# david-cortes/cmfrec

Hardware: AMD Instinct MI355X
Metric: ALS rows/sec ((users+items)/iteration time), implicit ALS-CG k=50 fp64 (higher is better)
Workload: dtype f64

## Files before the change

cmfrec_amd/csrc/cg_kernels.hpp:

```cpp
#pragma once
#include <hip/hip_runtime.h>
#include <stdint.h>
#include <type_traits>

#include "lanes.hpp"

namespace cmfhip {

constexpr int WAVE = 64;
constexpr int TILE = 64;
constexpr int MAX_W = 8;
#ifndef CMF_CG_WAVES_PER_SIMD
#define CMF_CG_WAVES_PER_SIMD 2
#endif
#ifndef CMF_CG_WAVES_PER_SIMD_F32
#define CMF_CG_WAVES_PER_SIMD_F32 3
#endif
#ifndef CMF_CG_WAVES_PER_SIMD_LOW
#define CMF_CG_WAVES_PER_SIMD_LOW 3
#endif
constexpr int CG_NTSEL_MAX_S = 7;
template <typename T, int W, int NRES_, int NTSEL = 0> constexpr int cg_waves_per_simd()
{
    if (sizeof(T) == 8 && NTSEL == 1 && W <= 8) return CMF_CG_WAVES_PER_SIMD_LOW;
// ... 110 lines not shown
#pragma unroll
        for (int s = 0; s < S; s++) tile.set(t, s, val);
}

template <typename T>
__device__ __forceinline__ T wave_sum(T v) { return lanes::wave_sum(v); }

template <typename T, int NT, int I>
__device__ __forceinline__ T treduce8_low_first(const T (&v)[8], bool h)
{
    if constexpr (I + 4 < NT) {
        T keep = h ? v[I + 4] : v[I];
        return keep + lanes::recv_xor4(v[I], v[I + 4]);
    } else return v[I] + lanes::xor4_lower(v[I]);
}
template <typename T, int NT = 8>
__device__ __forceinline__ T treduce8_low(const T (&v)[8], int lane)
{
    static_assert(NT >= 4 && NT <= 8, "entries per lane group");
    T u[4], q[2];
    bool h = (lane & 4) != 0;
    u[0] = treduce8_low_first<T, NT, 0>(v, h); u[1] = treduce8_low_first<T, NT, 1>(v, h);
    u[2] = treduce8_low_first<T, NT, 2>(v, h); u[3] = treduce8_low_first<T, NT, 3>(v, h);
    h = (lane & 2) != 0;
#pragma unroll
    for (int i = 0; i < 2; i++) {
        T keep = h ? u[i + 2] : u[i];
        T send = h ? u[i] : u[i + 2];
        q[i] = keep + lanes::xor2(send);
    }
    h = (lane & 1) != 0;
    T keep = h ? q[1] : q[0];
    T send = h ? q[0] : q[1];
    return keep + lanes::xor1(send);
}

template <typename T>
__device__ __forceinline__ T treduce8_high(const T (&v)[8], int lane)
{
    T u[4], q[2];
#pragma unroll
    for (int i = 0; i < 4; i++) u[i] = lanes::tswap32_add(v[i], v[i + 4]);
#pragma unroll
    for (int i = 0; i < 2; i++) q[i] = lanes::tswap16_add(u[i], u[i + 2]);
    const bool h = (lane & 8) != 0;
    T keep = h ? q[1] : q[0];
    return keep + lanes::recv_xor8(q[0], q[1]);
}

#ifndef CMF_PASS_VECTOR_LDS
#define CMF_PASS_VECTOR_LDS 2
#endif
template <typename T> constexpr bool pass_vector_in_lds() { return CMF_PASS_VECTOR_LDS == 1 || (CMF_PASS_VECTOR_LDS == 2 && sizeof(T) == 8); }
template <typename T, int S>
__device__ __forceinline__ void replicate(T vdist, T (&vrep)[S], int lane);
template <typename T, int S, int GR = 8>
__device__ __forceinline__ void pass_vector_lds(T vdist, T (&vrep)[S], T (&wts)[8], int lane, T *__restrict__ pv)
{
    const int jj = lane >> 3, ll = lane & 7;
    pv[lane] = vdist;
    __builtin_amdgcn_wave_barrier();
#pragma unroll
    for (int s = 0; s < S; s++) vrep[s] = pv[ll + 8 * s];
    const T *wp = pv + GR * jj;
#pragma unroll
    for (int t = 0; t < GR; t++) wts[t] = wp[t];
    __builtin_amdgcn_wave_barrier();
}

__host__ __device__ constexpr int gram_ld(int S) { return 8 * S + 1; }
#ifndef CMF_GRAM_ROWS_BY_K
#define CMF_GRAM_ROWS_BY_K 1
#endif
template <typename T> __host__ __device__ constexpr int gram_rows(int S) { return (CMF_GRAM_ROWS_BY_K && pass_vector_in_lds<T>()) ? S : 8; }
__host__ __device__ constexpr int gram_ld_rows(int S, int GR)
{
    if (GR == 8) return gram_ld(S);
    int ld = 8 * S;
    while ((S * ld) % 32 != 8 && (S * ld) % 32 != 24) ld++;
    return ld;
}
__host__ __device__ constexpr int gram_ld2(int S) { return 8 * S + 2; }
template <typename T> __host__ __device__ constexpr int gram_elems(int S) { return sizeof(T) == 4 ? 64 * gram_ld2(S) : 64 * gram_ld(S); }
template <typename T, int S, int GR = 8> __device__ __forceinline__ int gram_index(int r, int c)
{
    if constexpr (sizeof(T) == 4) return 2 * ((r >> 1) * gram_ld2(S) + c) + (r & 1);
    else return r * gram_ld_rows(S, GR) + c;
}
template <typename T, int S, int GR = 8>
__device__ __forceinline__ void stage_gramian(T *__restrict__ G, const T *__restrict__ BtB, int k, int tid, int nthreads)
{
    static_assert(GR == 8 || sizeof(T) == 8, "rows by k: double precision");
    for (int e = tid; e < 8 * GR * 8 * S; e += nthreads) {
        const int r = e / (8 * S), c = e % (8 * S);
        G[gram_index<T, S, GR>(r, c)] = (r < k && c < k) ? BtB[(size_t)r * k + c] : T(0);
    }
}

template <typename T, int S>
struct RegTile {
    T v[8][S];
    __device__ __forceinline__ void set(int t, int s, T x) { v[t][s] = x; }
};
typedef float f32x2 __attribute__((ext_vector_type(2)));
template <int S>
struct RegTile<float, S> {
    f32x2 v[4][S];
    __device__ __forceinline__ void set(int t, int s, float x) { v[t >> 1][s][t & 1] = x; }
};

template <typename T>
struct PassAcc {
    T v[8];
    __device__ __forceinline__ void zero()
    {
#pragma unroll
        for (int s = 0; s < 8; s++) v[s] = T(0);
    }
    __device__ __forceinline__ void close(T (&out)[8]) const
    {
#pragma unroll
        for (int s = 0; s < 8; s++) out[s] = v[s];
    }
};
template <>
struct PassAcc<float> {
    f32x2 v[8];
    __device__ __forceinline__ void zero()
    {
#pragma unroll
        for (int s = 0; s < 8; s++) v[s] = f32x2{0.f, 0.f};
    }
    __device__ __forceinline__ void close(float (&out)[8]) const
    {
#pragma unroll
        for (int s = 0; s < 8; s++) out[s] = v[s][0] + v[s][1];
    }
};

template <typename T, int S, int NT = 8>
__device__ __forceinline__ void load_tile(RegTile<T, S> &tile, const T *__restrict__ Bm, size_t ldb,
                                          int k, int my_idx, int cnt, int lane)
{
    const int jj = lane >> 3, ll = lane & 7;
    int its[8];
    its[0] = lanes::bcast8<0>(my_idx); its[1] = lanes::bcast8<1>(my_idx); its[2] = lanes::bcast8<2>(my_idx);
    its[3] = lanes::bcast8<3>(my_idx);
    if (NT > 4) its[4] = lanes::bcast8<4>(my_idx);
    if (NT > 5) its[5] = lanes::bcast8<5>(my_idx);
    if (NT > 6) its[6] = lanes::bcast8<6>(my_idx);
    if (NT > 7) its[7] = lanes::bcast8<7>(my_idx);
    const int first_idx = __builtin_amdgcn_readfirstlane(my_idx);
    const int col_last = min(ll + 8 * (S - 1), k - 1) - ll;
    const char *base = reinterpret_cast<const char *>(Bm + ll);
    const unsigned ldb_bytes = (unsigned)(ldb * sizeof(T));
#pragma unroll
    for (int t = 0; t < NT; t++) {
        const unsigned it = (unsigned)(((jj * NT + t) < cnt) ? its[t] : first_idx);
        const T *rp = reinterpret_cast<const T *>(base + (unsigned long long)it * ldb_bytes);
#pragma unroll
        for (int s = 0; s < S; s++) tile.set(t, s, rp[(s < S - 1) ? 8 * s : col_last]);
    }
}

template <typename T, bool IMPLICIT, int MODE>
__device__ __forceinline__ T pass_weight(T coef, T x, bool valid, T g = T(1))
// ... 85 lines not shown
        for (int s = S; s < 8; s++) out.v[s] = T(0);
    }
    }
}

template <typename T, int S, int W>
__device__ __forceinline__ void gram_pass(const T *__restrict__ G, T wdist, PassAcc<T> &out, int lane, int wr)
{
    constexpr int LD = gram_ld(S);
    const int jj = lane >> 3, ll = lane & 7;
    T wts[8];
    wts[0] = lanes::bcast8<0>(wdist); wts[1] = lanes::bcast8<1>(wdist); wts[2] = lanes::bcast8<2>(wdist);
    wts[3] = lanes::bcast8<3>(wdist); wts[4] = lanes::bcast8<4>(wdist); wts[5] = lanes::bcast8<5>(wdist);
    wts[6] = lanes::bcast8<6>(wdist); wts[7] = lanes::bcast8<7>(wdist);
    if constexpr (std::is_same<T, float>::value && W <= 4) {
#pragma unroll
        for (int q = 0; q < 4; q++) {
            if (W > 1 && (q % W) != wr) continue;
            const f32x2 *g = reinterpret_cast<const f32x2 *>(G) + (jj * 4 + q) * gram_ld2(S) + ll;
            const f32x2 w2 = f32x2{wts[2 * q], wts[2 * q + 1]};
#pragma unroll
            for (int s = 0; s < S; s++) out.v[s] += w2 * lds_g(g + 8 * s);
        }
    } else {
#pragma unroll
        for (int t = 0; t < 8; t++) {
            if (W > 1 && (t % W) != wr) continue;
#pragma unroll
            for (int s = 0; s < S; s++) {
                if constexpr (std::is_same<T, float>::value) out.v[s][0] += wts[t] * G[gram_index<T, S>(jj * 8 + t, ll + 8 * s)];
                else out.v[s] += wts[t] * lds_g(G + (jj * 8 + t) * LD + ll + 8 * s);
            }
        }
    }
}

template <bool NEG, typename T, int S, int W, int GR = 8>
__device__ __forceinline__ void gram_pass_w(const T *__restrict__ G, const T (&wts)[8], PassAcc<T> &out, int lane, int wr)
{
    constexpr int LD = gram_ld_rows(S, GR);
    const int jj = lane >> 3, ll = lane & 7;
    if constexpr (std::is_same<T, float>::value && W <= 4) {
#pragma unroll
        for (int q = 0; q < 4; q++) {
            if (W > 1 && (q % W) != wr) continue;
            const f32x2 *g = reinterpret_cast<const f32x2 *>(G) + (jj * 4 + q) * gram_ld2(S) + ll;
            const f32x2 w2 = f32x2{wts[2 * q], wts[2 * q + 1]};
#pragma unroll
            for (int s = 0; s < S; s++) out.v[s] = NEG ? out.v[s] - w2 * lds_g(g + 8 * s) : out.v[s] + w2 * lds_g(g + 8 * s);
        }
    } else {
#pragma unroll
        for (int t = 0; t < GR; t++) {
            if (W > 1 && (t % W) != wr) continue;
#pragma unroll
            for (int s = 0; s < S; s++) {
                if constexpr (std::is_same<T, float>::value) {
                    const float g = G[gram_index<T, S>(jj * 8 + t, ll + 8 * s)];
                    out.v[s][0] = NEG ? out.v[s][0] - wts[t] * g : out.v[s][0] + wts[t] * g;
                } else {
                    const T g = lds_g(G + (jj * GR + t) * LD + ll + 8 * s);
                    out.v[s] = NEG ? out.v[s] - wts[t] * g : out.v[s] + wts[t] * g;
                }
            }
        }
    }
}

template <typename T, int S>
__device__ __forceinline__ void replicate(T vdist, T (&vrep)[S], int lane)
{
    const int ll = lane & 7;
#pragma unroll
    for (int s = 0; s < S; s++) vrep[s] = __shfl(vdist, s * 8 + ll);
}

template <typename T, int S, bool IMPLICIT, int W, int RPB, bool GRAMX = false, int NRES_ = 0, int NTSEL = 0>
__global__ void __launch_bounds__(64 * W * RPB, (cg_waves_per_simd<T, W, NRES_, NTSEL>()))
cg_rows_kernel(const CgParams<T> P)
{
    constexpr bool GRAM = IMPLICIT || GRAMX;
    extern __shared__ __attribute__((aligned(16))) unsigned char smem_raw[];
    T *G = reinterpret_cast<T *>(smem_raw);
    T *red = G + (GRAM ? gram_elems<T>(S) : 0);
    const int tid = threadIdx.x;
    const int lane = tid & 63;
    const int wave = tid >> 6;
    const int grp = wave / W;
    const int wr = wave % W;
    const int k = P.k;

    const int nteams = gridDim.x * RPB;
    __shared__ int s_claim[4];
    constexpr bool PV = pass_vector_in_lds<T>();
    __shared__ __attribute__((aligned(16))) T s_pv[PV ? W * RPB : 1][PV ? 64 : 1];
    const int cslot = (blockIdx.x * RPB + grp) % CG_NCOUNTERS;
    int *const my_counter = P.counter + cslot * CG_COUNTER_STRIDE;
    const int cbase = nteams + cslot;
    auto issue_claim = [&]() -> int {
        int v = 0;
        if (wr == 0 && lane == 0) v = atomicAdd(my_counter, 1);
        return v;
    };
    int rnxt, rnn;
    if (W == 1) {
        const int c1 = issue_claim(), c2 = issue_claim();
        rnxt = cbase + CG_NCOUNTERS * __builtin_amdgcn_readfirstlane(c1);
        rnn = cbase + CG_NCOUNTERS * __builtin_amdgcn_readfirstlane(c2);
    } else if (wr == 0 && lane == 0) {
        s_claim[2] = cbase + CG_NCOUNTERS * atomicAdd(my_counter, 1);
        s_claim[3] = cbase + CG_NCOUNTERS * atomicAdd(my_counter, 1);
    }
    constexpr int GR = gram_rows<T>(S);
    if (GRAM) stage_gramian<T, S, GR>(G, P.BtB, k, tid, blockDim.x);
    if (GRAM || W > 1) __syncthreads();
    if (W > 1) { rnxt = s_claim[2]; rnn = s_claim[3]; }
    T *myred = red + (size_t)grp * 2 * W * 64;

    int buf = 0;
    static_assert(W == 1 || RPB == 1, "multi-wave teams own their workgroup (barriers are per row)");

    constexpr int NRES = NRES_ > 0 ? NRES_ : ((std::is_same<T, float>::value && W == 8) ? 2 : 1);
    static_assert(NRES == 1 || std::is_same<T, float>::value, "two resident tiles: single precision");
    static_assert(NTSEL == 0 || (S >= CMF_CG_NT_MIN_S && (sizeof(T) == 4 || S <= CG_NTSEL_MAX_S) && NRES_ == 0),
                  "launches by tile size: tiles by row length (double precision: k <= 56)");
    constexpr int NT_MIN = (S >= CMF_CG_NT_MIN_S && (CMF_CG_NT_F32 || !std::is_same<T, float>::value)) ? (std::is_same<T, float>::value ? 6 : 5) : 8;
    auto nt_of = [&](int nnz_) -> int {
        int nt = (nnz_ + 8 * W * NRES - 1) / (8 * W * NRES);
        if (std::is_same<T, float>::value) nt = (nt + 1) & ~1;
        return (nt > 8) ? 8 : (nt < NT_MIN ? NT_MIN : nt);
    };
    struct Pre { int idx; T x; T a; int idx2; T x2; T g; T g2; };
    auto load_desc = [&](int rix_) -> RowDesc {
        RowDesc d; d.row = 0; d.nnz = 0; d.st = 0;
        if (rix_ < P.nrows) d = P.desc[rix_];
        d.row = __builtin_amdgcn_readfirstlane(d.row);
        d.nnz = __builtin_amdgcn_readfirstlane(d.nnz);
        d.st = ((unsigned long long)(unsigned)__builtin_amdgcn_readfirstlane((int)(d.st >> 32)) << 32) |
               (unsigned)__builtin_amdgcn_readfirstlane((int)(d.st & 0xffffffffu));
        return d;
    };
    auto load_pre = [&](const RowDesc &d) -> Pre {
        Pre q; q.idx = 0; q.x = T(0); q.a = T(0); q.idx2 = 0; q.x2 = T(0); q.g = T(1); q.g2 = T(1);
        const int nt = nt_of(d.nnz), tl = 8 * nt;
        const int b = lane & 7;
        const int ent = (lane >> 3) * nt + b;
        const int cnt = min(tl, d.nnz - wr * tl);
        if (b < nt && ent < cnt) {
            const size_t pos = d.st + (size_t)wr * tl + ent;
            q.idx = P.indices[pos];
            q.x = P.values[pos];
            q.g = entry_weight<T, IMPLICIT>(P, pos);
            if (!IMPLICIT && P.bias_sub != nullptr) q.x -= P.bias_sub[q.idx];
        }
        if (NRES == 2) {
            const int cnt2 = min(tl, d.nnz - (wr + W) * tl);
            if (b < nt && ent < cnt2) {
                const size_t pos = d.st + (size_t)(wr + W) * tl + ent;
                q.idx2 = P.indices[pos];
                q.x2 = P.values[pos];
                q.g2 = entry_weight<T, IMPLICIT>(P, pos);
                if (!IMPLICIT && P.bias_sub != nullptr) q.x2 -= P.bias_sub[q.idx2];
            }
        }
        if (d.nnz > 0 && lane < k) q.a = P.A[(size_t)d.row * P.lda + lane];
        return q;
    };
    int rix = blockIdx.x * RPB + grp;
    RowDesc dcur = load_desc(rix);
    RowDesc dnxt = load_desc(rnxt);
    Pre pcur = load_pre(dcur);
    int pend = issue_claim();
#ifdef CMF_CG_TICKS
    unsigned long long tk_wait = 0, tk_pass = 0, tk_rows = 0;
    const unsigned long long tk_begin = CMF_TICK();
#endif
    int it = 0;
    RowDesc dnn;
    Pre pnxt;
    auto solve_row = [&](auto nt_tag) {
        constexpr int NT = decltype(nt_tag)::value;
        constexpr int TL = 8 * NT;
        const int row = dcur.row;
        const size_t st = dcur.st;
        const int nnz = dcur.nnz;
        const int ntiles = (nnz + TL - 1) / TL;
        const int my_ntiles = (ntiles > wr) ? (ntiles - wr + W - 1) / W : 0;
        const bool resident = NT < 8 || my_ntiles <= NRES;

        T lam = P.lam, lam_last = P.lam_last;
        if (GRAMX && P.kc > 0) {
            if (P.scale_lam || P.scale_lam_sideinfo) {
                T mult = row_lam_mult(P, row, nnz);
                if (P.scale_lam_sideinfo) mult += (T)P.p_side;
                lam *= mult; lam_last *= mult;
            }
        } else if (!IMPLICIT && P.scale_lam) {
            const T mult = row_lam_mult(P, row, nnz);
            lam *= mult;
            if (!P.scale_bias_const) lam_last *= mult;
        }
        T *arow = P.A + (size_t)row * P.lda;
        T a_d = pcur.a;

        RegTile<T, S> tile;
        const int ent = (lane >> 3) * NT + (lane & 7);
        const bool lane_has = (NT == 8) || (lane & 7) < NT;
        const int cnt0 = min(TL, nnz - wr * TL);
        T x_res = pcur.x;
        const T g_res = pcur.g;
        bool valid_res = lane_has && ent < cnt0;
        if (CMF_DBG(P, 1)) dbg_fill_tile<8, S>(tile, (T)(pcur.idx & 3) * (T)0.001);
        else if (cnt0 > 0) load_tile<T, S, NT>(tile, P.B, P.ldb, k, pcur.idx, cnt0, lane);
        RegTile<T, (NRES == 2) ? S : 1> tile2;
        const int cnt1 = (NRES == 2) ? min(TL, nnz - (wr + W) * TL) : 0;
        const T x2_res = pcur.x2, g2_res = pcur.g2;
        const bool valid2_res = lane_has && ent < cnt1;
        if constexpr (NRES == 2) {
            if (cnt1 > 0 && !CMF_DBG(P, 1)) load_tile<T, S, NT>(tile2, P.B, P.ldb, k, pcur.idx2, cnt1, lane);
        }
        dnn = load_desc(rnn);
        pnxt = load_pre(dnxt);
#ifdef CMF_CG_TICKS
        const unsigned long long tk0 = CMF_TICK();
        asm volatile("s_waitcnt vmcnt(0)" ::: "memory");
        const unsigned long long tk1 = CMF_TICK();
        tk_wait += tk1 - tk0;
#endif

        auto run_pass = [&](T vdist, auto mode_tag, bool first) -> T {
            constexpr int MODE = decltype(mode_tag)::value;
            asm volatile("" ::: "memory");
            T vrep[S];
            T gw[8];
            if constexpr (PV) pass_vector_lds<T, S, GR>(vdist, vrep, gw, lane, &s_pv[wave][0]);
            else replicate<T, S>(vdist, vrep, lane);
            PassAcc<T> acc;
            acc.zero();
            if constexpr (NRES == 2) {
                if (cnt0 > 0 && !CMF_DBG(P, 4)) tile_pass<T, S, IMPLICIT, MODE, NT>(tile, vrep, x_res, valid_res, acc, lane, g_res);
                if (cnt1 > 0 && !CMF_DBG(P, 4)) tile_pass<T, S, IMPLICIT, MODE, NT>(tile2, vrep, x2_res, valid2_res, acc, lane, g2_res);
            } else if constexpr (NT < 8) {
                if (cnt0 > 0 && !CMF_DBG(P, 4)) tile_pass<T, S, IMPLICIT, MODE, NT>(tile, vrep, x_res, valid_res, acc, lane, g_res);
            } else
            for (int tl = wr; tl < ntiles; tl += W) {
                T x, g; bool valid;
                const bool have = (tl == wr) && (resident || first);
                if (!have) {
                    const int cnt = min(TL, nnz - tl * TL);
                    valid = lane_has && ent < cnt;
                    const size_t pos = st + (size_t)tl * TL + ent;
                    int my_idx = valid ? P.indices[pos] : 0;
                    x = valid ? P.values[pos] : T(0);
                    g = valid ? entry_weight<T, IMPLICIT>(P, pos) : T(1);
                    if (!IMPLICIT && P.bias_sub != nullptr && valid) x -= P.bias_sub[my_idx];
                    if (!CMF_DBG(P, 1)) load_tile<T, S, NT>(tile, P.B, P.ldb, k, my_idx, cnt, lane);
                } else {
                    x = x_res; g = g_res; valid = valid_res;
                }
                if (!CMF_DBG(P, 4)) tile_pass<T, S, IMPLICIT, MODE, NT>(tile, vrep, x, valid, acc, lane, g);
            }
            if (GRAM && !CMF_DBG(P, 2)) {
                if constexpr (PV) gram_pass_w<MODE == 0, T, S, W, GR>(G, gw, acc, lane, wr);
                else gram_pass<T, S, W>(G, (MODE == 0) ? -vdist : vdist, acc, lane, wr);
            }
            T out[8];
            acc.close(out);
            T tot = treduce8_high<T>(out, lane);
            if (W > 1) {
                T *rb = myred + (size_t)buf * W * 64;
                rb[wr * 64 + lane] = tot;
                if (first && wr == 0 && lane == 0) s_claim[it & 1] = cbase + CG_NCOUNTERS * pend;
                __syncthreads();
                tot = T(0);
#pragma unroll
                for (int w = 0; w < W; w++) tot += rb[w * 64 + lane];
                buf ^= 1;
            }
            return tot;
        };

        T r_d = run_pass(a_d, std::integral_constant<int, 0>{}, true);
        r_d -= lam * a_d;
        if (!IMPLICIT && lam != lam_last && lane == k - 1) r_d -= (lam_last - lam) * a_d;
        if (GRAMX && P.rconst != nullptr && lane < k) r_d += P.rconst[(size_t)row * P.ldr + lane];
        if (lane >= k) r_d = T(0);
        T p_d = r_d;
        T r_old = CMF_DBG(P, 8) ? T(1) : wave_sum(r_d * r_d);
        bool done = (r_old <= (T)1e-12);
        for (int step = 0; step < P.max_cg_steps && !done; step++) {
            T Ap_d = run_pass(p_d, std::integral_constant<int, 1>{}, false);
            Ap_d += lam * p_d;
            if (!IMPLICIT && lam != lam_last && lane == k - 1) Ap_d += (lam_last - lam) * p_d;
            if (lane >= k) Ap_d = T(0);
            T alpha = CMF_DBG(P, 8) ? T(0.001) : cg_div(r_old, wave_sum(Ap_d * p_d));
            a_d += alpha * p_d;
            r_d -= alpha * Ap_d;
            T r_new = CMF_DBG(P, 8) ? T(0.5) : wave_sum(r_d * r_d);
            if (r_new <= (T)1e-8) done = true;
            else {
                p_d = p_d * cg_div(r_new, r_old) + r_d;
                r_old = r_new;
            }
        }
        if (wr == 0 && lane < k) arow[lane] = a_d;
#ifdef CMF_CG_TICKS
        tk_pass += CMF_TICK() - tk1; tk_rows += (wr == 0);
#endif
    };
    for (; rix < P.nrows; it++) {
        const int nt = nt_of(dcur.nnz);
        if constexpr (NT_MIN == 8) solve_row(std::integral_constant<int, 8>{});
        else if constexpr (std::is_same<T, float>::value) {
            if constexpr (NTSEL == 1) solve_row(std::integral_constant<int, 6>{});
            else if constexpr (NTSEL == 2) solve_row(std::integral_constant<int, 8>{});
            else if (nt == 6) solve_row(std::integral_constant<int, 6>{});
            else solve_row(std::integral_constant<int, 8>{});
        } else if constexpr (NTSEL == 1) {
            if (nt <= 5) solve_row(std::integral_constant<int, 5>{});
            else solve_row(std::integral_constant<int, 6>{});
        } else if constexpr (NTSEL == 2) {
            if (nt <= 7) solve_row(std::integral_constant<int, 7>{});
            else solve_row(std::integral_constant<int, 8>{});
        } else {
            switch (nt) {
                case 5: solve_row(std::integral_constant<int, 5>{}); break;
                case 6: solve_row(std::integral_constant<int, 6>{}); break;
                case 7: solve_row(std::integral_constant<int, 7>{}); break;
                default: solve_row(std::integral_constant<int, 8>{}); break;
            }
        }
        const int r3 = (W == 1) ? cbase + CG_NCOUNTERS * __builtin_amdgcn_readfirstlane(pend) : s_claim[it & 1];
        dcur = dnxt; dnxt = dnn; pcur = pnxt;
        rix = rnxt; rnxt = rnn; rnn = r3;
        pend = issue_claim();
    }
#ifdef CMF_CG_TICKS
    cg_ticks_flush(P.ticks, W == 1 ? 0 : W == 2 ? 1 : W == 4 ? 2 : 3, tk_wait, tk_pass, tk_rows, CMF_TICK() - tk_begin, lane);
#endif
}

constexpr int TILE4 = 32;

template <typename T, int S>
struct RegTile4 {
    T v[4][S];
    __device__ __forceinline__ void set(int t, int s, T x) { v[t][s] = x; }
    __device__ __forceinline__ T get(int t, int s) const { return v[t][s]; }
};
template <int S>
struct RegTile4<float, S> {
    f32x2 v[2][S];
    __device__ __forceinline__ void set(int t, int s, float x) { v[t >> 1][s][t & 1] = x; }
    __device__ __forceinline__ f32x2 pair0(int s) const { return v[0][s]; }
};

template <typename T, int S>
__device__ __forceinline__ void load_tile4(RegTile4<T, S> &tile, const T *__restrict__ Bm, size_t ldb,
                                           int k, int my_idx, int cnt, int lane)
{
    const int jj = lane >> 3, ll = lane & 7;
    int its[4];
    its[0] = lanes::bcast8<0>(my_idx); its[1] = lanes::bcast8<2>(my_idx);
    its[2] = lanes::bcast8<4>(my_idx); its[3] = lanes::bcast8<6>(my_idx);
    const int first_idx = __builtin_amdgcn_readfirstlane(my_idx);
    const int col_last = min(ll + 8 * (S - 1), k - 1) - ll;
    const char *base = reinterpret_cast<const char *>(Bm + ll);
    const unsigned ldb_bytes = (unsigned)(ldb * sizeof(T));
#pragma unroll
    for (int t = 0; t < 4; t++) {
        const unsigned it = (unsigned)(((jj * 4 + t) < cnt) ? its[t] : first_idx);
        const T *rp = reinterpret_cast<const T *>(base + (unsigned long long)it * ldb_bytes);
#pragma unroll
        for (int s = 0; s < S; s++) tile.set(t, s, rp[(s < S - 1) ? 8 * s : col_last]);
    }
}

template <typename T>
__device__ __forceinline__ T treduce4_low(const T (&v)[4], int lane)
{
    T u[2];
    bool h = (lane & 4) != 0;
#pragma unroll
    for (int i = 0; i < 2; i++) {
        T keep = h ? v[i + 2] : v[i];
        u[i] = keep + lanes::recv_xor4(v[i], v[i + 2]);
    }
    h = (lane & 2) != 0;
    T keep = h ? u[1] : u[0];
    T send = h ? u[0] : u[1];
    T q = keep + lanes::xor2(send);
    return q + lanes::xor1(q);
}

template <int S, bool IMPLICIT, int MODE, typename TILE, bool INIT = false>
__device__ __forceinline__ void tile_pass4_f32(const TILE &tile, const float (&vrep)[S], float x, bool valid,
                                           PassAcc<float> &out, int lane, float g = 1.f)
{
    float c[4];
#pragma unroll
    for (int q = 0; q < 2; q++) {
        f32x2 acc = f32x2{0.f, 0.f};
#pragma unroll
        for (int s = 0; s < S; s++) acc += tile.v[q][s] * f32x2{vrep[s], vrep[s]};
        c[2 * q] = acc[0]; c[2 * q + 1] = acc[1];
    }
    float coef = treduce4_low<float>(c, lane);
    const float w = pass_weight<float, IMPLICIT, MODE>(coef, x, valid, g);
    float wts[4];
    wts[0] = lanes::bcast8<0>(w); wts[1] = lanes::bcast8<2>(w); wts[2] = lanes::bcast8<4>(w); wts[3] = lanes::bcast8<6>(w);
#pragma unroll
    for (int q = 0; q < 2; q++) {
        const f32x2 w2 = f32x2{wts[2 * q], wts[2 * q + 1]};
#pragma unroll
        for (int s = 0; s < S; s++) out.v[s] = (INIT && q == 0) ? w2 * tile.v[q][s] : out.v[s] + w2 * tile.v[q][s];
    }
    if constexpr (INIT) {
#pragma unroll
// ... 854 lines not shown
```

cmfrec_amd/csrc/device.hpp:

```cpp
#pragma once
#include <hip/hip_runtime.h>
#include <algorithm>
#include <cstdio>
#include <cstdlib>
#include <cstring>
#include <numeric>
#include <string>
#include <vector>

#include "../../include/cmfrec_hip.h"
#include "cg_kernels.hpp"
#include "chol_kernels.hpp"
#include "dense_kernels.hpp"
#include "gram_cg_kernels.hpp"
#include "topn_kernels.hpp"

namespace cmfhip {

extern thread_local std::string g_last_error;

struct HipError {
    int code;
};

inline void hip_check(hipError_t e, const char *what, const char *file, int line)
{
    if (e == hipSuccess) return;
    char buf[512];
    snprintf(buf, sizeof buf, "cmfrec_hip: %s failed: %s (%s:%d)", what, hipGetErrorString(e), file, line);
    g_last_error = buf;
    fprintf(stderr, "%s\n", buf);
    throw HipError{e == hipErrorOutOfMemory ? 1 : 4};
}
#define HIP_CHECK(x) ::cmfhip::hip_check((x), #x, __FILE__, __LINE__)

struct Switches {
    bool poison_lds = false;
    int vh_min = 0;
    int vh = 0;
    bool gram_slice = false;
    int bins_par = 2;
    bool nt_split = true;
    bool cg_generic = false;
    int chol = 0;
    int parts_coop = 1;
    int chol_wg = 2;
    int gramk = -1;
    int gramk_batch = 0;
    int lowrank = -1;
    bool eig_jacobi = false;
    int debug_skip = 0;
    bool debug_ticks = false;
    void reload()
    {
        auto str = [](const char *n) -> const char * { const char *v = getenv(n); return (v != nullptr && v[0] != 0) ? v : nullptr; };
        auto num = [&](const char *n, int dflt) -> int { const char *v = str(n); return v ? atoi(v) : dflt; };
        poison_lds = str("CMFREC_HIP_POISON_LDS") != nullptr;
        vh_min = num("CMFREC_HIP_VH_MIN", 0);
        const char *v = str("CMFREC_HIP_VH");
        vh = !v ? 0 : strcmp(v, "stream") == 0 ? 1 : strcmp(v, "gram") == 0 ? 2 : 1;
        v = str("CMFREC_HIP_GRAM_KERNEL"); gram_slice = v && strcmp(v, "slice") == 0;
        bins_par = num("CMFREC_HIP_BINS_PAR", 2);
        nt_split = num("CMFREC_HIP_NT_SPLIT", 1) != 0;
        v = str("CMFREC_HIP_CG_KERNEL"); cg_generic = v && strcmp(v, "generic") == 0;
        v = str("CMFREC_HIP_CHOL"); chol = !v ? 0 : strcmp(v, "rows") == 0 ? 1 : strcmp(v, "noslices") == 0 ? 2 : 0;
        parts_coop = num("CMFREC_HIP_PARTS_COOP", 1);
        chol_wg = num("CMFREC_HIP_CHOL_WG", 2);
        if (chol_wg == 1) chol_wg = 2;
        gramk = num("CMFREC_HIP_GRAMK", -1);
        gramk_batch = num("CMFREC_HIP_GRAMK_BATCH", 0);
        lowrank = num("CMFREC_HIP_LOWRANK", -1);
        v = str("CMFREC_HIP_EIG"); eig_jacobi = v && strcmp(v, "jacobi") == 0;
        debug_skip = num("CMFREC_HIP_CG_SKIP", num("CMFREC_HIP_CHOL_SKIP", num("CMFREC_HIP_WAVE_SKIP", 0)));
        debug_ticks = str("CMFREC_HIP_GRAM_TICKS") != nullptr || str("CMFREC_HIP_CHOL_TICKS") != nullptr;
    }
};
inline Switches &switches_mut() { static Switches sw; static bool first = (sw.reload(), true); (void)first; return sw; }
inline const Switches &switches() { return switches_mut(); }

template <typename T>
struct DevBuf {
    T *ptr = nullptr;
    size_t n = 0;
    bool owned = true;
    DevBuf() = default;
    DevBuf(const DevBuf &) = delete;
    DevBuf &operator=(const DevBuf &) = delete;
    ~DevBuf() { release(); }
    void release()
    {
        if (ptr && owned) (void)hipFree(ptr);
        ptr = nullptr;
        n = 0;
    }
    void alloc(size_t count)
    {
        release();
        n = count;
        owned = true;
        if (count) HIP_CHECK(hipMalloc((void **)&ptr, count * sizeof(T)));
        if (count && switches().poison_lds) {
            HIP_CHECK(hipMemset(ptr, 0xFF, count * sizeof(T)));
            HIP_CHECK(hipDeviceSynchronize());
        }
    }
    void alloc_at_least(size_t count)
    {
        if (n < count) alloc(count);
    }
    void upload(const T *host, size_t count, hipStream_t st)
    {
        if (count > n) alloc(count);
        if (count) HIP_CHECK(hipMemcpyAsync(ptr, host, count * sizeof(T), hipMemcpyDefault, st));
    }
    void download(T *host, size_t count, hipStream_t st) const
    {
        if (count) HIP_CHECK(hipMemcpyAsync(host, ptr, count * sizeof(T), hipMemcpyDeviceToHost, st));
    }
};

constexpr int MAX_DEVICES = 16;
constexpr int NBINS = 6;
constexpr int BIN_VHEAVY = 0;
constexpr int BIN_HEAVY = 1;
constexpr int BIN_MED4 = 2;
constexpr int BIN_MED2 = 3;
constexpr int BIN_LIGHT = 4;
constexpr int BIN_TINY = 5;
constexpr int BIN_MIN_NNZ[NBINS] = {1025, 257, 129, 65, 33, 1};
inline int vh_min_env()
{
    const int v = switches().vh_min;
    return v > 0 ? std::min(sizeof(real_t) == 4 ? BIN_MIN_NNZ[BIN_VHEAVY] : (1 << 30), std::max(258, v)) : 0;
}

struct SparseShard {
    int nrows = 0;
    size_t nnz = 0;
    int vh_min = BIN_MIN_NNZ[BIN_VHEAVY];
    size_t opp_row_bytes_hint = 50 * sizeof(real_t);
    int bin_of(long long l) const
    {
        if (l >= vh_min) return BIN_VHEAVY;
        for (int b = 1; b < NBINS; b++)
            if (l >= BIN_MIN_NNZ[b]) return b;
        return -1;
// ... 313 lines not shown
        }
        hipLaunchKernelGGL(gram_reduce_kernel<real_t>, dim3((k * k + GRAM_RED_ENT - 1) / GRAM_RED_ENT), dim3(256), 0, dev.stream,
                           ws.partial.ptr, nblocks, k * k, out, scale, add_diag, k);
    } else {
        launch_gemm<true>(dev, k, k, n, scale, B, ldb, B, ldb, out, (size_t)k);
        if (add_diag != 0)
            hipLaunchKernelGGL(add_diag_kernel<real_t>, dim3((k + 255) / 256), dim3(256), 0, dev.stream, out, k, 0, k, add_diag);
    }
    HIP_CHECK(hipGetLastError());
}

struct CgCall {
    real_t *A; size_t lda;
    const real_t *B; size_t ldb;
    int k;
    const real_t *bias_sub;
    const real_t *BtB;
    real_t lam, lam_last;
    bool scale_lam, scale_bias_const;
    int max_cg_steps;
    bool implicit;
    bool precond = false;
    int koff = 0, kc = 0;
    const real_t *CtC = nullptr, *UC = nullptr;
    real_t w_side = 0;
    int rows_with_u = 0, p_side = 0;
    bool scale_lam_sideinfo = false;
    const SparseShard *X2 = nullptr;
    const real_t *C2 = nullptr;
    const real_t *Bi = nullptr, *BiTBi = nullptr;
    int ki = 0;
    real_t w_imp = 0;
    const real_t *gsum = nullptr;
    int skip_first = 0;
    const real_t *Gx = nullptr, *rconst_x = nullptr;
    size_t ldr_x = 0;
    const real_t *values_override = nullptr, *weights_override = nullptr;
    bool gx_all_rows = false;
    const real_t *wsum_override = nullptr;
};

enum class CgVariant { Auto, Generic };
CgVariant cg_variant_from_env();

constexpr int NCOUNTER_SETS = 2 * NBINS + 2;
constexpr size_t ROW_COUNTER_INTS = 64 + (size_t)NCOUNTER_SETS * CG_NCOUNTERS * CG_COUNTER_STRIDE;
inline size_t cg_counter_offset(int bin) { return 64 + (size_t)bin * CG_NCOUNTERS * CG_COUNTER_STRIDE; }

__global__ void __launch_bounds__(256) poison_lds_kernel(int words)
{
    extern __shared__ unsigned int poison_words[];
    volatile unsigned int *w = poison_words;
    for (int e = threadIdx.x; e < words; e += 256) w[e] = 0xFFFFFFFFu;
}
inline void poison_lds(hipStream_t st, int num_cus)
{
    if (!switches().poison_lds) return;
    constexpr int BYTES = 80 * 1024;
    static thread_local bool attr_set = false;
    if (!attr_set) {
        HIP_CHECK(hipFuncSetAttribute((const void *)poison_lds_kernel, hipFuncAttributeMaxDynamicSharedMemorySize, BYTES));
        attr_set = true;
    }
    hipLaunchKernelGGL(poison_lds_kernel, dim3(num_cus * 4), dim3(256), BYTES, st, BYTES / 4);
    HIP_CHECK(hipGetLastError());
}

template <int S, bool IMPLICIT, int W, int RPB, bool GRAMX = false, int NRES_ = 0, int NTSEL = 0>
inline void launch_cg_bin(const DeviceInfo &dev, CgParams<real_t> P, int first, int count, BinTimers *tm, int bin, hipStream_t st, int counter_set = -1)
{
    if (count <= 0) return;
    EventPair ev{nullptr, nullptr};
    if (tm) {
        HIP_CHECK(hipEventCreate(&ev.a));
        HIP_CHECK(hipEventCreate(&ev.b));
        HIP_CHECK(hipEventRecord(ev.a, st));
    }
    poison_lds(st, dev.num_cus);
    P.order += first;
    P.desc += first;
    P.nrows = count;
    P.counter = dev.row_counter.ptr + cg_counter_offset(counter_set >= 0 ? counter_set : bin);
    constexpr int threads = 64 * W * RPB;
    size_t smem = (((IMPLICIT || GRAMX) ? (size_t)gram_elems<real_t>(S) : 0) + (size_t)RPB * 2 * W * 64) * sizeof(real_t);
    auto kern = cg_rows_kernel<real_t, S, IMPLICIT, W, RPB, GRAMX, NRES_, NTSEL>;
    static thread_local int bpc_dev[MAX_DEVICES] = {0};
    int &blocks_per_cu = bpc_dev[std::min(std::max(dev.device, 0), MAX_DEVICES - 1)];
    if (blocks_per_cu == 0) {
        if (smem > 48 * 1024)
            HIP_CHECK(hipFuncSetAttribute((const void *)kern, hipFuncAttributeMaxDynamicSharedMemorySize, (int)smem));
        int nb = 0;
        HIP_CHECK(hipOccupancyMaxActiveBlocksPerMultiprocessor(&nb, kern, threads, smem));
        blocks_per_cu = std::max(1, nb);
    }
    int teams_needed = (count + RPB - 1) / RPB;
    int grid = std::min(teams_needed, dev.num_cus * blocks_per_cu);
    hipLaunchKernelGGL(kern, dim3(grid), dim3(threads), smem, st, P);
    HIP_CHECK(hipGetLastError());
    if (tm) {
        HIP_CHECK(hipEventRecord(ev.b, st));
        tm->ev[bin].push_back(ev);
    }
}

template <int S, bool IMPLICIT, bool GRAMX = false>
inline void launch_cg_tiny(const DeviceInfo &dev, CgParams<real_t> P, int first, int count, BinTimers *tm, hipStream_t st, int n_gt16)
{
    if (count <= 0) return;
    EventPair ev{nullptr, nullptr};
    if (tm) {
        HIP_CHECK(hipEventCreate(&ev.a));
        HIP_CHECK(hipEventCreate(&ev.b));
        HIP_CHECK(hipEventRecord(ev.a, st));
    }
    poison_lds(st, dev.num_cus);
    constexpr bool tiny16_on = true;
    const int count_le16 = std::min(count, std::max(0, first + count - std::max(first, n_gt16)));
    size_t smem = ((IMPLICIT || GRAMX) ? (size_t)gram_elems<real_t>(S) : 0) * sizeof(real_t);
    const int di = std::min(std::max(dev.device, 0), MAX_DEVICES - 1);
    CgParams<real_t> P1 = P;
    P1.order += first;
    P1.desc += first;
    P1.nrows = count;
    P1.counter = dev.row_counter.ptr + cg_counter_offset(BIN_TINY);
    {
        const bool mixed = tiny16_on && count_le16 > 0;
        auto kern = mixed ? cg_rows_tiny_kernel<real_t, S, IMPLICIT, GRAMX, 0> : cg_rows_tiny_kernel<real_t, S, IMPLICIT, GRAMX, 4>;
        static thread_local int bpc_dev[MAX_DEVICES][2] = {{0}};
        int &blocks_per_cu = bpc_dev[di][mixed ? 1 : 0];
        if (blocks_per_cu == 0) {
            int nb = 0;
            HIP_CHECK(hipOccupancyMaxActiveBlocksPerMultiprocessor(&nb, kern, 256, smem));
            blocks_per_cu = std::max(1, nb);
        }
        const int grid = std::min((count + 3) / 4, dev.num_cus * blocks_per_cu);
        hipLaunchKernelGGL(kern, dim3(grid), dim3(256), smem, st, P1);
    }
    HIP_CHECK(hipGetLastError());
    if (tm) {
        HIP_CHECK(hipEventRecord(ev.b, st));
        tm->ev[BIN_TINY].push_back(ev);
    }
}

void launch_gram_wave(dim3 grid, hipStream_t st, const CgParams<real_t> &P, const GramParams<real_t> &G, bool implicit, int rem);

template <bool GRAMX>
inline bool vh_takes_gram(int k, const SparseShard &X)
{
    if (GRAMX || k > 16 * GRAM_NTT) return false;
    return (switches().vh != 0) ? switches().vh == 2 : X.prefer_gram((size_t)k * sizeof(real_t));
}

template <int S, bool IMPLICIT, bool GRAMX = false>
inline void launch_cg_vheavy(const DeviceInfo &dev_, CgParams<real_t> P, const SparseShard &X, BinTimers *tm, hipStream_t st)
{
    const int nvh = X.bin_rows[BIN_VHEAVY];
    if (nvh <= 0) return;
    struct { hipStream_t stream; int num_cus; } dev{st, dev_.num_cus};
    EventPair ev{nullptr, nullptr};
    if (tm) {
        HIP_CHECK(hipEventCreate(&ev.a));
        HIP_CHECK(hipEventCreate(&ev.b));
        HIP_CHECK(hipEventRecord(ev.a, dev.stream));
    }
    if (vh_takes_gram<GRAMX>(P.k, X)) {
        GramParams<real_t> G;
        G.sl_vrow = X.sl_vrow.ptr; G.sl_first = X.sl_first.ptr; G.sl_count = X.sl_count.ptr; G.row_sl_off = X.row_sl_off.ptr;
        G.part = X.gram_part.ptr; G.n_slices = X.n_slices; G.nvh = nvh;
        P.nrows = nvh;
#ifdef CMF_CG_DEBUG
        if (switches().debug_ticks) {
            static unsigned long long *d_t = nullptr;
            unsigned long long h[4];
            if (d_t == nullptr) { HIP_CHECK(hipMalloc((void **)&d_t, sizeof(h))); HIP_CHECK(hipMemset(d_t, 0, sizeof(h))); }
            else {
                HIP_CHECK(hipDeviceSynchronize());
                HIP_CHECK(hipMemcpy(h, d_t, sizeof(h), hipMemcpyDeviceToHost));
                if (h[1] > 0)
                    fprintf(stderr, "gram_wave: %.0f ticks per wave, %llu waves, %llu slices, %llu nnz: %.1f ticks per nnz and wave\n",
                            (double)h[0] / h[1], h[1], h[2], h[3], (double)h[0] / (double)h[3]);
                HIP_CHECK(hipMemset(d_t, 0, sizeof(h)));
            }
            G.ticks = d_t;
        }
#endif
        poison_lds(dev.stream, dev.num_cus);
        const bool slice_kernel = switches().gram_slice;
        if (slice_kernel)
            hipLaunchKernelGGL((gram_slice_kernel<real_t, IMPLICIT>), dim3(std::min(X.n_slices, dev.num_cus * 2)), dim3(64 * GRAM_NW), 0,
                           dev.stream, P, G);
        else {
            const dim3 gw(std::min((X.n_slices + 3) / 4, dev.num_cus * 4));
            const int rem = (sizeof(real_t) == 8) ? P.k - 16 * (GRAM_NTT - 1) : 0;
            launch_gram_wave(gw, dev.stream, P, G, IMPLICIT, rem);
        }
        poison_lds(dev.stream, dev.num_cus);
        hipLaunchKernelGGL((gram_cg_kernel<real_t, IMPLICIT>), dim3(std::min(nvh, dev.num_cus * 8)), dim3(256), 0, dev.stream, P, G);
        HIP_CHECK(hipGetLastError());
        if (tm) {
            HIP_CHECK(hipEventRecord(ev.b, dev.stream));
            tm->ev[BIN_VHEAVY].push_back(ev);
        }
        return;
    }
    VhState<real_t> V;
    V.r = X.vh_r.ptr; V.p = X.vh_p.ptr; V.r_old = X.vh_r_old.ptr; V.done = X.vh_done.ptr; V.part = X.vh_part.ptr;
    V.chunk_row = X.vh_chunk_row.ptr; V.chunk_start = X.vh_chunk_start.ptr; V.chunk_cnt = X.vh_chunk_cnt.ptr;
    V.chunk_off = X.vh_chunk_off.ptr; V.launch = X.vh_launch.ptr; V.work = X.vh_work.ptr;
    V.nvh = nvh; V.nchunks = X.n_chunks; V.nlaunch = X.n_launch;
    P.nrows = nvh;
    poison_lds(dev.stream, dev.num_cus);
    const dim3 gp(X.n_launch), bp(64 * VH_CHUNK_TILES), gu(nvh), bu(64 * VH_UPD_WAVES);
    hipLaunchKernelGGL((vh_pass_kernel<real_t, S, IMPLICIT, 0>), gp, bp, 0, dev.stream, P, V);
    hipLaunchKernelGGL((vh_update_kernel<real_t, IMPLICIT, 0, GRAMX>), gu, bu, 0, dev.stream, P, V);
    for (int step = 0; step < P.max_cg_steps; step++) {
        hipLaunchKernelGGL((vh_pass_kernel<real_t, S, IMPLICIT, 1>), gp, bp, 0, dev.stream, P, V);
        hipLaunchKernelGGL((vh_update_kernel<real_t, IMPLICIT, 1, GRAMX>), gu, bu, 0, dev.stream, P, V);
    }
    HIP_CHECK(hipGetLastError());
    if (tm) {
        HIP_CHECK(hipEventRecord(ev.b, dev.stream));
        tm->ev[BIN_VHEAVY].push_back(ev);
    }
}

inline int cg_bin_streams()
{
    const int n = switches().bins_par;
    return std::min(std::max(n, 1), DeviceInfo::MAX_BIN_STREAMS + 1);
}

template <int S, bool IMPLICIT, int W, int RPB, bool GRAMX>
inline void launch_cg_bin_by_tile(const DeviceInfo &dev, const CgParams<real_t> &P, const SparseShard &X, int first, int count, BinTimers *tm, int bin,
                                  hipStream_t st)
{
#ifdef CMFREC_HIP_FLOAT
    constexpr bool by_tile = S >= CMF_CG_NT_MIN_S && CMF_CG_NT_F32 && W <= 4;
#else
    constexpr bool by_tile = S >= CMF_CG_NT_MIN_S && S <= CG_NTSEL_MAX_S && (W == 1 || W == 4 || W == 8);
#endif
    if (count <= 0) return;
    if constexpr (by_tile) {
        if (switches().nt_split) {
            const int n_hi = std::min(count, std::max(0, X.n_gt_low[W == 1 ? 0 : W == 2 ? 1 : W == 4 ? 2 : 3] - first));
            EventPair ev{nullptr, nullptr};
            if (tm) { HIP_CHECK(hipEventCreate(&ev.a)); HIP_CHECK(hipEventCreate(&ev.b)); HIP_CHECK(hipEventRecord(ev.a, st)); }
            launch_cg_bin<S, IMPLICIT, W, RPB, GRAMX, 0, 2>(dev, P, first, n_hi, nullptr, bin, st);
            launch_cg_bin<S, IMPLICIT, W, RPB, GRAMX, 0, 1>(dev, P, first + n_hi, count - n_hi, nullptr, bin, st, NBINS + 2 + bin);
            if (tm) { HIP_CHECK(hipEventRecord(ev.b, st)); tm->ev[bin].push_back(ev); }
            return;
        }
    }
    launch_cg_bin<S, IMPLICIT, W, RPB, GRAMX>(dev, P, first, count, tm, bin, st);
}

template <int S, bool IMPLICIT, bool GRAMX>
inline void launch_cg_any_bin(const DeviceInfo &dev, const CgParams<real_t> &P, const SparseShard &X, BinTimers *tm, int bin, hipStream_t st)
{
    const int first = X.bin_first[bin], count = X.bin_rows[bin];
    switch (bin) {
        case BIN_HEAVY:
#ifdef CMFREC_HIP_FLOAT
            {
                const int n_long8 = std::min(count, std::max(0, X.n_gt512 - first));
                EventPair ev{nullptr, nullptr};
                if (tm) { HIP_CHECK(hipEventCreate(&ev.a)); HIP_CHECK(hipEventCreate(&ev.b)); HIP_CHECK(hipEventRecord(ev.a, st)); }
                launch_cg_bin<S, IMPLICIT, 8, 1, GRAMX>(dev, P, first, n_long8, nullptr, bin, st);
                launch_cg_bin<S, IMPLICIT, 4, 1, GRAMX, 2>(dev, P, first + n_long8, count - n_long8, nullptr, bin, st, NBINS);
                if (tm) { HIP_CHECK(hipEventRecord(ev.b, st)); tm->ev[bin].push_back(ev); }
                break;
            }
#endif
            launch_cg_bin_by_tile<S, IMPLICIT, 8, 1, GRAMX>(dev, P, X, first, count, tm, bin, st); break;
        case BIN_MED4: launch_cg_bin_by_tile<S, IMPLICIT, 4, 1, GRAMX>(dev, P, X, first, count, tm, bin, st); break;
        case BIN_MED2: launch_cg_bin_by_tile<S, IMPLICIT, 2, 1, GRAMX>(dev, P, X, first, count, tm, bin, st); break;
        default: launch_cg_bin_by_tile<S, IMPLICIT, 1, 4, GRAMX>(dev, P, X, first, count, tm, bin, st); break;
    }
}

template <int S, bool IMPLICIT, bool GRAMX = false>
inline void launch_cg_S(const DeviceInfo &dev, const CgParams<real_t> &P, const SparseShard &X, BinTimers *tm)
{
    if (dev.row_counter.n < ROW_COUNTER_INTS) const_cast<DeviceInfo &>(dev).row_counter.alloc(ROW_COUNTER_INTS);
    HIP_CHECK(hipMemsetAsync(dev.row_counter.ptr, 0, ROW_COUNTER_INTS * sizeof(int), dev.stream));
    const bool vh_aside = X.bin_rows[BIN_VHEAVY] > 0 && X.vh_runs_aside(dev.num_cus) && !vh_takes_gram<GRAMX>(P.k, X);
    const bool alt = X.is_part;
    DeviceInfo &d = const_cast<DeviceInfo &>(dev);
    const int npar = cg_bin_streams();
    if (npar > 1 && !(vh_aside || alt)) {
        d.ensure_bin_streams(npar - 1);
        hipStream_t ss[DeviceInfo::MAX_BIN_STREAMS + 1];
        ss[0] = dev.stream;
        for (int i = 1; i < npar; i++) ss[i] = d.bin_streams[i - 1];
        HIP_CHECK(hipEventRecord(d.fork_ev, dev.stream));
        for (int i = 1; i < npar; i++) HIP_CHECK(hipStreamWaitEvent(ss[i], d.fork_ev, 0));
        static const double row_equiv[NBINS] = {0.0, 126.0, 7.0, 7.0, 0.0, 11.5};
        double cost[NBINS], load[DeviceInfo::MAX_BIN_STREAMS + 1] = {0, 0, 0, 0, 0, 0};
        int order_b[NBINS];
        for (int b = 0; b < NBINS; b++) {
            cost[b] = (double)X.bin_nnz[b] + row_equiv[b] * (double)X.bin_rows[b];
            order_b[b] = b;
        }
        std::sort(order_b, order_b + NBINS, [&](int a, int b2) { return cost[a] > cost[b2]; });
        for (int q = 0; q < NBINS; q++) {
            const int b = order_b[q];
            if (X.bin_rows[b] <= 0) continue;
            int si = 0;
            for (int i = 1; i < npar; i++) if (load[i] < load[si]) si = i;
            load[si] += cost[b];
            if (b == BIN_VHEAVY) launch_cg_vheavy<S, IMPLICIT, GRAMX>(dev, P, X, tm, ss[si]);
            else if (b == BIN_TINY) launch_cg_tiny<S, IMPLICIT, GRAMX>(dev, P, X.bin_first[BIN_TINY], X.bin_rows[BIN_TINY], tm, ss[si], X.n_gt16);
            else launch_cg_any_bin<S, IMPLICIT, GRAMX>(dev, P, X, tm, b, ss[si]);
        }
        for (int i = 1; i < npar; i++) {
            HIP_CHECK(hipEventRecord(d.bin_join[i - 1], ss[i]));
            HIP_CHECK(hipStreamWaitEvent(dev.stream, d.bin_join[i - 1], 0));
        }
        return;
    }
    if (vh_aside || alt) {
        d.ensure_aux();
        HIP_CHECK(hipEventRecord(d.fork_ev, dev.stream));
        HIP_CHECK(hipStreamWaitEvent(d.aux_stream, d.fork_ev, 0));
    }
    hipStream_t s0 = dev.stream, s1 = alt ? d.aux_stream : dev.stream;
    launch_cg_vheavy<S, IMPLICIT, GRAMX>(dev, P, X, tm, (vh_aside || (alt && X.is_part)) ? d.aux_stream : dev.stream);
    launch_cg_any_bin<S, IMPLICIT, GRAMX>(dev, P, X, tm, BIN_HEAVY, s0);
    launch_cg_any_bin<S, IMPLICIT, GRAMX>(dev, P, X, tm, BIN_MED4, s1);
    launch_cg_any_bin<S, IMPLICIT, GRAMX>(dev, P, X, tm, BIN_MED2, s0);
    launch_cg_any_bin<S, IMPLICIT, GRAMX>(dev, P, X, tm, BIN_LIGHT, s1);
    launch_cg_tiny<S, IMPLICIT, GRAMX>(dev, P, X.bin_first[BIN_TINY], X.bin_rows[BIN_TINY], tm, s0, X.n_gt16);
// ... 179 lines not shown
```

Before: 168.7 million.

## Allow two multi-wave CG teams per workgroup for medium-row bins, with a tighter Gramian LDS footprint

Lets multi-wave CG teams share a workgroup (RPB>1). Each team gets its own claim slots, and a liveness handshake keeps the per-row block barriers matched until every team has finished. It adds an optional path that runs W=2 low-tile rows as team pairs, gated behind a new env switch that is off by default. It also shrinks the staged Gramian LDS allocation to the size actually indexed for double precision, which could raise blocks per CU everywhere. The risk is that the team pairs share __syncthreads, so one team stalls on the other's rows.

```diff
diff --git a/cmfrec_amd/csrc/cg_kernels.hpp b/cmfrec_amd/csrc/cg_kernels.hpp
--- a/cmfrec_amd/csrc/cg_kernels.hpp
+++ b/cmfrec_amd/csrc/cg_kernels.hpp
@@ -216,6 +216,11 @@
 }
 __host__ __device__ constexpr int gram_ld2(int S) { return 8 * S + 2; }
 template <typename T> __host__ __device__ constexpr int gram_elems(int S) { return sizeof(T) == 4 ? 64 * gram_ld2(S) : 64 * gram_ld(S); }
+template <typename T> __host__ __device__ constexpr int gram_staged_elems(int S)
+{
+    return sizeof(T) == 4 ? gram_elems<T>(S) : 8 * gram_rows<T>(S) * gram_ld_rows(S, gram_rows<T>(S));
+}
+static_assert(gram_staged_elems<double>(7) == 56 * 56 && gram_staged_elems<double>(7) <= gram_elems<double>(7), "staged Gramian, k = 50");
 template <typename T, int S, int GR = 8> __device__ __forceinline__ int gram_index(int r, int c)
 {
     if constexpr (sizeof(T) == 4) return 2 * ((r >> 1) * gram_ld2(S) + c) + (r & 1);
@@ -467,16 +472,19 @@
     constexpr bool GRAM = IMPLICIT || GRAMX;
     extern __shared__ __attribute__((aligned(16))) unsigned char smem_raw[];
     T *G = reinterpret_cast<T *>(smem_raw);
-    T *red = G + (GRAM ? gram_elems<T>(S) : 0);
+    T *red = G + (GRAM ? gram_staged_elems<T>(S) : 0);
     const int tid = threadIdx.x;
     const int lane = tid & 63;
-    const int wave = tid >> 6;
+    const int wave = (W > 1 && RPB > 1) ? __builtin_amdgcn_readfirstlane(tid >> 6) : tid >> 6;
     const int grp = wave / W;
     const int wr = wave % W;
     const int k = P.k;
 
     const int nteams = gridDim.x * RPB;
-    __shared__ int s_claim[4];
+    __shared__ int s_claim[RPB][4];
+    const int cteam = (RPB > 1) ? grp : 0;
+    constexpr bool TEAMS = W > 1 && RPB > 1;
+    __shared__ int s_live[TEAMS ? 2 : 1][TEAMS ? RPB : 1];
     constexpr bool PV = pass_vector_in_lds<T>();
     __shared__ __attribute__((aligned(16))) T s_pv[PV ? W * RPB : 1][PV ? 64 : 1];
     const int cslot = (blockIdx.x * RPB + grp) % CG_NCOUNTERS;
@@ -493,17 +501,20 @@
         rnxt = cbase + CG_NCOUNTERS * __builtin_amdgcn_readfirstlane(c1);
         rnn = cbase + CG_NCOUNTERS * __builtin_amdgcn_readfirstlane(c2);
     } else if (wr == 0 && lane == 0) {
-        s_claim[2] = cbase + CG_NCOUNTERS * atomicAdd(my_counter, 1);
-        s_claim[3] = cbase + CG_NCOUNTERS * atomicAdd(my_counter, 1);
+        s_claim[cteam][2] = cbase + CG_NCOUNTERS * atomicAdd(my_counter, 1);
+        s_claim[cteam][3] = cbase + CG_NCOUNTERS * atomicAdd(my_counter, 1);
+    }
+    if constexpr (TEAMS) {
+        if (tid < 2 * RPB) s_live[tid / RPB][tid % RPB] = 1;
     }
     constexpr int GR = gram_rows<T>(S);
     if (GRAM) stage_gramian<T, S, GR>(G, P.BtB, k, tid, blockDim.x);
     if (GRAM || W > 1) __syncthreads();
-    if (W > 1) { rnxt = s_claim[2]; rnn = s_claim[3]; }
+    if (W > 1) { rnxt = s_claim[cteam][2]; rnn = s_claim[cteam][3]; }
     T *myred = red + (size_t)grp * 2 * W * 64;
 
     int buf = 0;
-    static_assert(W == 1 || RPB == 1, "multi-wave teams own their workgroup (barriers are per row)");
+    static_assert(64 * W * RPB <= 1024, "workgroup size");
 
     constexpr int NRES = NRES_ > 0 ? NRES_ : ((std::is_same<T, float>::value && W == 8) ? 2 : 1);
     static_assert(NRES == 1 || std::is_same<T, float>::value, "two resident tiles: single precision");
@@ -655,7 +666,7 @@
             if (W > 1) {
                 T *rb = myred + (size_t)buf * W * 64;
                 rb[wr * 64 + lane] = tot;
-                if (first && wr == 0 && lane == 0) s_claim[it & 1] = cbase + CG_NCOUNTERS * pend;
+                if (first && wr == 0 && lane == 0) s_claim[cteam][it & 1] = cbase + CG_NCOUNTERS * pend;
                 __syncthreads();
                 tot = T(0);
 #pragma unroll
@@ -715,10 +726,21 @@
                 default: solve_row(std::integral_constant<int, 8>{}); break;
             }
         }
-        const int r3 = (W == 1) ? cbase + CG_NCOUNTERS * __builtin_amdgcn_readfirstlane(pend) : s_claim[it & 1];
+        const int r3 = (W == 1) ? cbase + CG_NCOUNTERS * __builtin_amdgcn_readfirstlane(pend) : s_claim[cteam][it & 1];
         dcur = dnxt; dnxt = dnn; pcur = pnxt;
         rix = rnxt; rnxt = rnn; rnn = r3;
         pend = issue_claim();
+    }
+    if constexpr (TEAMS) {
+        for (;;) {
+            if (wr == 0 && lane == 0) s_live[buf][grp] = 0;
+            __syncthreads();
+            int live = 0;
+#pragma unroll
+            for (int g = 0; g < RPB; g++) live |= s_live[buf][g];
+            buf ^= 1;
+            if (__builtin_amdgcn_readfirstlane(live) == 0) break;
+        }
     }
 #ifdef CMF_CG_TICKS
     cg_ticks_flush(P.ticks, W == 1 ? 0 : W == 2 ? 1 : W == 4 ? 2 : 3, tk_wait, tk_pass, tk_rows, CMF_TICK() - tk_begin, lane);
diff --git a/cmfrec_amd/csrc/device.hpp b/cmfrec_amd/csrc/device.hpp
--- a/cmfrec_amd/csrc/device.hpp
+++ b/cmfrec_amd/csrc/device.hpp
@@ -41,6 +41,7 @@
     bool gram_slice = false;
     int bins_par = 2;
     bool nt_split = true;
+    bool med2_pairs = false;
     bool cg_generic = false;
     int chol = 0;
     int parts_coop = 1;
@@ -62,6 +63,7 @@
         v = str("CMFREC_HIP_GRAM_KERNEL"); gram_slice = v && strcmp(v, "slice") == 0;
         bins_par = num("CMFREC_HIP_BINS_PAR", 2);
         nt_split = num("CMFREC_HIP_NT_SPLIT", 1) != 0;
+        med2_pairs = num("CMFREC_HIP_MED2_PAIRS", 0) != 0;
         v = str("CMFREC_HIP_CG_KERNEL"); cg_generic = v && strcmp(v, "generic") == 0;
         v = str("CMFREC_HIP_CHOL"); chol = !v ? 0 : strcmp(v, "rows") == 0 ? 1 : strcmp(v, "noslices") == 0 ? 2 : 0;
         parts_coop = num("CMFREC_HIP_PARTS_COOP", 1);
@@ -541,7 +543,7 @@
     P.nrows = count;
     P.counter = dev.row_counter.ptr + cg_counter_offset(counter_set >= 0 ? counter_set : bin);
     constexpr int threads = 64 * W * RPB;
-    size_t smem = (((IMPLICIT || GRAMX) ? (size_t)gram_elems<real_t>(S) : 0) + (size_t)RPB * 2 * W * 64) * sizeof(real_t);
+    size_t smem = (((IMPLICIT || GRAMX) ? (size_t)gram_staged_elems<real_t>(S) : 0) + (size_t)RPB * 2 * W * 64) * sizeof(real_t);
     auto kern = cg_rows_kernel<real_t, S, IMPLICIT, W, RPB, GRAMX, NRES_, NTSEL>;
     static thread_local int bpc_dev[MAX_DEVICES] = {0};
     int &blocks_per_cu = bpc_dev[std::min(std::max(dev.device, 0), MAX_DEVICES - 1)];
@@ -696,8 +698,14 @@
 {
 #ifdef CMFREC_HIP_FLOAT
     constexpr bool by_tile = S >= CMF_CG_NT_MIN_S && CMF_CG_NT_F32 && W <= 4;
+    constexpr int RPB_LOW = RPB;
 #else
-    constexpr bool by_tile = S >= CMF_CG_NT_MIN_S && S <= CG_NTSEL_MAX_S && (W == 1 || W == 4 || W == 8);
+    constexpr bool pairs = W == 2 && IMPLICIT && !GRAMX;
+    constexpr bool by_tile = S >= CMF_CG_NT_MIN_S && S <= CG_NTSEL_MAX_S && (W == 1 || W == 4 || W == 8 || pairs);
+    constexpr int RPB_LOW = pairs ? 2 : RPB;
+    if constexpr (pairs) {
+        if (!switches().med2_pairs) { launch_cg_bin<S, IMPLICIT, W, RPB, GRAMX>(dev, P, first, count, tm, bin, st); return; }
+    }
 #endif
     if (count <= 0) return;
     if constexpr (by_tile) {
@@ -706,7 +714,7 @@
             EventPair ev{nullptr, nullptr};
             if (tm) { HIP_CHECK(hipEventCreate(&ev.a)); HIP_CHECK(hipEventCreate(&ev.b)); HIP_CHECK(hipEventRecord(ev.a, st)); }
             launch_cg_bin<S, IMPLICIT, W, RPB, GRAMX, 0, 2>(dev, P, first, n_hi, nullptr, bin, st);
-            launch_cg_bin<S, IMPLICIT, W, RPB, GRAMX, 0, 1>(dev, P, first + n_hi, count - n_hi, nullptr, bin, st, NBINS + 2 + bin);
+            launch_cg_bin<S, IMPLICIT, W, RPB_LOW, GRAMX, 0, 1>(dev, P, first + n_hi, count - n_hi, nullptr, bin, st, NBINS + 2 + bin);
             if (tm) { HIP_CHECK(hipEventRecord(ev.b, st)); tm->ev[bin].push_back(ev); }
             return;
         }
```

Result: no change. 169.9 million, median of 6 (+0.7%).
